# ssilverman16/particle_col_image_segmentation

Hardware: AMD Instinct MI355X
Metric: Mpixels/sec segmented (5-ch 1024x1024 TIFF), ROI mask IoU=1.0 (higher is better)
Workload: dtype f32 planes / u8 class maps / int32 labels / f64 ROI sums; 1 GPU; BASELINE config 2: batch of 64 frames 1024x1024x5 float32 per GPU, full kernel chain, inputs resident in HBM; frames_per_gpu=64, height=1024, width=1024, planes=5, parallelism=frames x1, launch=one hipGraph replay per step, 4 in flight, tie_fallback_frames_last_step=0, reference_nan_frames_rank0=0

## Files before the change

particle_col_image_segmentation_amd/csrc/ccl.hip:

```cpp
#include <type_traits>

#include "column_pass.h"
#include "tile_ops.h"

namespace pcseg {

constexpr int SCAN_PIX = 1024;

struct KeyEqU8 {
    const uint8_t *p;
    int W;
    int64_t n;
    __device__ __forceinline__ int operator()(int b, int r, int c) const { return p[b * n + rowoff(r, W) + c]; }
};
struct KeyNzU8 {
    const uint8_t *p;
    int W;
    int64_t n;
    __device__ __forceinline__ int operator()(int b, int r, int c) const { return p[b * n + rowoff(r, W) + c] != 0; }
};
struct KeyZeroU8 {
    const uint8_t *p;
    int W;
    int64_t n;
    __device__ __forceinline__ int operator()(int b, int r, int c) const { return p[b * n + rowoff(r, W) + c] == 0; }
};
struct KeyIsOneU8 {
    const uint8_t *p;
    int W;
    int64_t n;
    __device__ __forceinline__ int operator()(int b, int r, int c) const { return p[b * n + rowoff(r, W) + c] == 1; }
};
struct KeyI32 {
    const int32_t *p;
    int W;
    int64_t n;
    __device__ __forceinline__ int operator()(int b, int r, int c) const { return p[b * n + rowoff(r, W) + c]; }
};
__device__ __forceinline__ bool cand_bit(const unsigned long long *bits, int64_t g) { return (bits[g >> 6] >> (g & 63)) & 1ull; }
struct KeyCandBits {
    const int32_t *img;
    const unsigned long long *bits;
    int W;
    int64_t n;
    __device__ __forceinline__ int operator()(int b, int r, int c) const
    {
        const int64_t g = b * n + rowoff(r, W) + c;
        if (!cand_bit(bits, g)) return 0;
        const int v = img[g];
        return v == 0 ? (int)0x80000000 : v;
    }
};
struct KeyBits {
    const unsigned *words;
    int W, nch;
    __device__ __forceinline__ int operator()(int b, int r, int c) const
    {
        return (words[((int64_t)b * nch + (r >> 5)) * W + c] >> (r & 31)) & 1u;
    }
};

template <typename KeyFn, bool CONN8>
__global__ void __launch_bounds__(256) ccl_tile_kernel(KeyFn keyfn, int *__restrict__ parent, int H, int W)
{
    __shared__ int key[CCL_TILE];
    __shared__ int par[CCL_TILE];
    const int b = blockIdx.z, r0 = blockIdx.y * CCL_TH, c0 = blockIdx.x * CCL_TW;
    const int64_t fbase = (int64_t)b * H * W;
    if constexpr (std::is_same<KeyFn, KeyBits>::value) {
        const int lc = threadIdx.x % CCL_TW, c = c0 + lc;
        const unsigned word = c < W ? keyfn.words[((int64_t)b * keyfn.nch + (r0 >> 5)) * W + c] : 0u;
        for (int i = threadIdx.x; i < CCL_TILE; i += 256) {
            const int lr = i / CCL_TW;
            key[i] = (r0 + lr < H) ? (int)((word >> lr) & 1u) : 0;
        }
    } else {
        for (int i = threadIdx.x; i < CCL_TILE; i += 256) {
            int r = r0 + i / CCL_TW, c = c0 + i % CCL_TW;
            key[i] = (r < H && c < W) ? keyfn(b, r, c) : 0;
        }
    }
    __syncthreads();
    ccl_tile_unions<CONN8>(key, par);
    ccl_tile_store(key, par, parent, fbase, r0, c0, H, W);
}

template <typename KeyFn, bool CONN8>
__global__ void __launch_bounds__(256) ccl_border_kernel(KeyFn keyfn, int *__restrict__ parent, int H, int W, int *__restrict__ corrupt)
{
    const int n_top_rows = (H - 1) / CCL_TH, n_edges = (W - 1) / CCL_TW;
    const int n_cols = CONN8 ? 2 * n_edges : n_edges;
    int i = blockIdx.x * 256 + threadIdx.x;
    int r, c;
    if (i < n_top_rows * W) {
        r = (i / W + 1) * CCL_TH;
        c = i % W;
    } else {
        i -= n_top_rows * W;
        if (i >= n_cols * H) return;
        const int j = i / H;
        r = i % H;
        if ((r % CCL_TH) == 0 && r > 0) return;
        c = CONN8 ? ((j >> 1) + 1) * CCL_TW - (j & 1) : (j + 1) * CCL_TW;
    }
    const bool top = (r % CCL_TH) == 0 && r > 0;
    const bool left = (c % CCL_TW) == 0 && c > 0;
    const bool right = (c % CCL_TW) == CCL_TW - 1 && c + 1 < W;
    if (!top && !left && !(CONN8 && right && r > 0)) return;
    const int b = blockIdx.y;
    const int64_t fbase = (int64_t)b * H * W;
    int *par = parent + fbase;
    const int p = r * W + c;
    const int rn = max(r - 1, 0), cw = max(c - 1, 0), ce = min(c + 1, W - 1);
    const int k = keyfn(b, r, c);
    if (std::is_same<KeyFn, KeyCandBits>::value && k == 0) return;
    const int k_w = keyfn(b, r, cw), k_n = keyfn(b, rn, c), k_nw = keyfn(b, rn, cw), k_ne = CONN8 ? keyfn(b, rn, ce) : 0;
    if (k == 0) return;
    const bool w_same = c > 0 && k_w == k;
    const bool n_same = r > 0 && k_n == k;
    const bool nw_same = r > 0 && c > 0 && k_nw == k;
    const bool corner = top && left;
    int *bad = corrupt ? corrupt + b : nullptr;
    if (left && w_same && (corner || !(n_same && nw_same))) unite_glb(par, p, p - 1, bad);
    if (r > 0) {
        if (top && n_same && (corner || !(w_same && nw_same))) unite_glb(par, p, p - W, bad);
        if (CONN8) {
            if ((top || left) && nw_same && !n_same && !w_same) unite_glb(par, p, p - W - 1, bad);
            if (c + 1 < W && (top || right) && !n_same && k_ne == k) unite_glb(par, p, p - W + 1, bad);
        }
    }
}

struct PredAll {
    __device__ __forceinline__ bool operator()(int64_t) const { return true; }
};
struct PredNotFlagged {
    const uint8_t *flag;
    const int *frame_on;
    int64_t n;
    __device__ __forceinline__ bool operator()(int64_t gi) const { return flag[gi] == 0 && frame_on[gi / n] != 0; }
};

template <typename Pred>
__global__ void __launch_bounds__(256) ccl_flatten_count_kernel(int *__restrict__ parent, int *__restrict__ labels,
                                                                 int *__restrict__ blockcount, Pred pred, int64_t n, int nblk,
                                                                 bool flatten, int *__restrict__ corrupt)
{
    __shared__ int wsum[4];
    const int b = blockIdx.y;
    int *par = parent + (int64_t)b * n;
    int cnt = 0;
    const int64_t i0 = (int64_t)blockIdx.x * SCAN_PIX + threadIdx.x * 4;
    int pv[4] = {-1, -1, -1, -1};
    if ((n & 3) == 0 && i0 + 3 < n) {
        const int4 v = *reinterpret_cast<const int4 *>(par + i0);
        pv[0] = v.x; pv[1] = v.y; pv[2] = v.z; pv[3] = v.w;
    } else {
        for (int j = 0; j < 4; ++j)
            if (i0 + j < n) pv[j] = par[i0 + j];
    }
    bool isroot[4];
    for (int j = 0; j < 4; ++j) {
        const int64_t i = i0 + j;
        int p = pv[j];
        isroot[j] = false;
        if (i >= n || p < 0) continue;
        if (!walk_ok((int)i, p)) {
            walk_corrupt(corrupt ? corrupt + b : nullptr);
            continue;
        }
        if (flatten) {
            const int x = walk_root(par, p, corrupt ? corrupt + b : nullptr);
            if (x != p) par[i] = x;
            p = x;
        }
        isroot[j] = p == (int)i && pred((int64_t)b * n + i);
        cnt += isroot[j];
    }
    int total;
    int rank = block_exclusive_scan<256>(cnt, &total, wsum);
    for (int j = 0; j < 4; ++j)
        if (isroot[j]) labels[(int64_t)b * n + i0 + j] = -(++rank);
    if (threadIdx.x == 0) blockcount[b * nblk + blockIdx.x] = total;
}

__global__ void __launch_bounds__(256) ccl_scan_blocks_kernel(int *__restrict__ blockcount, int *__restrict__ counts, int nblk,
                                                               const int *__restrict__ corrupt)
{
    __shared__ int wsum[4];
    int *bc = blockcount + (int64_t)blockIdx.x * nblk;
    int carry = 0;
    for (int base = 0; base < nblk; base += 256) {
        int i = base + threadIdx.x;
        int v = i < nblk ? bc[i] : 0;
        int total;
        int ex = block_exclusive_scan<256>(v, &total, wsum);
        if (i < nblk) bc[i] = carry + ex;
        carry += total;
    }
    if (threadIdx.x == 0 && counts) counts[blockIdx.x] = (corrupt && corrupt[blockIdx.x]) ? -1 : carry;
}

template <typename Pred>
__global__ void __launch_bounds__(256) ccl_relabel_kernel(const int *__restrict__ parent, int *labels, const int *__restrict__ blockoff,
                                                           Pred pred, int64_t n, int nblk, bool chase, int *__restrict__ counts)
{
    const int b = blockIdx.y;
    const int *par = parent + (int64_t)b * n;
    int *lab = labels + (int64_t)b * n;
    const int64_t i0 = (int64_t)blockIdx.x * SCAN_PIX + threadIdx.x * 4;
    const bool vec = (n & 3) == 0 && i0 + 3 < n;
    int pv[4] = {-1, -1, -1, -1};
    if (vec) {
        const int4 v = *reinterpret_cast<const int4 *>(par + i0);
        pv[0] = v.x; pv[1] = v.y; pv[2] = v.z; pv[3] = v.w;
    } else {
        for (int j = 0; j < 4; ++j)
            if (i0 + j < n) pv[j] = par[i0 + j];
    }
    int out[4];
    int root_of_prev = -1, prev_p = -2;
    int bad = 0;
    for (int j = 0; j < 4; ++j) {
        int p = pv[j];
        int v = 0;
        if (p >= 0 && !walk_ok((int)(i0 + j), p)) {
            bad = 1;
            p = -1;
        }
        if (chase && p >= 0) {
            if (p == prev_p) {
                p = root_of_prev;
            } else {
                prev_p = p;
                p = walk_root(par, p, &bad);
                root_of_prev = p;
            }
        }
        if (p >= 0 && pred((int64_t)b * n + p)) {
            v = __hip_atomic_load(lab + p, __ATOMIC_RELAXED, __HIP_MEMORY_SCOPE_WORKGROUP);
            if (v < 0) v = blockoff[b * nblk + p / SCAN_PIX] - v;
        }
        out[j] = v;
    }
    if (vec) {
        *reinterpret_cast<int4 *>(lab + i0) = make_int4(out[0], out[1], out[2], out[3]);
    } else {
        for (int j = 0; j < 4; ++j)
            if (i0 + j < n) lab[i0 + j] = out[j];
    }
    if (bad && counts) counts[b] = -1;
}

constexpr int RELABEL_Q = 4;

template <typename Pred>
__device__ __forceinline__ int relabel_decode(const int *par, int *lab, const int *blockoff, const Pred &pred, int b, int64_t n, int nblk,
                                              int p, bool chase, int *bad)
{
    if (chase) p = walk_root(par, p, bad);
    if (!pred((int64_t)b * n + p)) return 0;
    int v = __hip_atomic_load(lab + p, __ATOMIC_RELAXED, __HIP_MEMORY_SCOPE_WORKGROUP);
    if (v < 0) v = blockoff[b * nblk + p / SCAN_PIX] - v;
    return v;
}

template <typename Pred, int NCH>
__device__ __forceinline__ void relabel_chains(const int *par, int *lab, const int *blockoff, const Pred &pred, int b, int64_t n, int nblk,
                                               bool chase, int (&root)[NCH], int (&val)[NCH], int *bad)
{
    if (chase) {
        bool more = true;
        while (more) {
            int nx[NCH];
#pragma unroll
            for (int q = 0; q < NCH; ++q) nx[q] = root[q] >= 0 ? par[root[q]] : -1;
            unsigned differ = 0, broke = 0;
#pragma unroll
            for (int q = 0; q < NCH; ++q) {
                const unsigned out = root[q] >= 0 && !walk_ok(root[q], nx[q]);
                broke |= out;
                nx[q] = out ? root[q] : nx[q];
                differ |= (unsigned)(nx[q] ^ root[q]);
// ... 23 lines not shown
{
    const int b = blockIdx.y;
    const int *par = parent + (int64_t)b * n;
    int *lab = labels + (int64_t)b * n;
    const int64_t i0 = (int64_t)blockIdx.x * (SCAN_PIX * RELABEL_Q) + threadIdx.x * 4;
    int4 pq[RELABEL_Q];
#pragma unroll
    for (int q = 0; q < RELABEL_Q; ++q) {
        const int64_t i = i0 + (int64_t)q * SCAN_PIX;
        pq[q] = i < n ? *reinterpret_cast<const int4 *>(par + i) : make_int4(-1, -1, -1, -1);
    }
    int bad = 0;
#pragma unroll
    for (int q = 0; q < RELABEL_Q; ++q) {
        const int i = (int)(i0 + (int64_t)q * SCAN_PIX);
        const int ox = pq[q].x >= 0 && !walk_ok(i, pq[q].x), oy = pq[q].y >= 0 && !walk_ok(i + 1, pq[q].y);
        const int oz = pq[q].z >= 0 && !walk_ok(i + 2, pq[q].z), ow = pq[q].w >= 0 && !walk_ok(i + 3, pq[q].w);
        bad |= ox | oy | oz | ow;
        pq[q].x = ox ? -1 : pq[q].x;
        pq[q].y = oy ? -1 : pq[q].y;
        pq[q].z = oz ? -1 : pq[q].z;
        pq[q].w = ow ? -1 : pq[q].w;
    }
    int lead[RELABEL_Q], lead2[RELABEL_Q], root[RELABEL_Q], val[RELABEL_Q], val2[RELABEL_Q], head_lane[RELABEL_Q];
    bool third = false;
    const int lane = lane_id();
#pragma unroll
    for (int q = 0; q < RELABEL_Q; ++q) {
        const int pv[4] = {pq[q].x, pq[q].y, pq[q].z, pq[q].w};
        lead[q] = pv[0] >= 0 ? pv[0] : (pv[1] >= 0 ? pv[1] : (pv[2] >= 0 ? pv[2] : pv[3]));
        const int left = __shfl_up(lead[q], 1);
        const bool head = lane == 0 || lead[q] != left;
        const unsigned long long heads = __ballot(head);
        head_lane[q] = 63 - __clzll((long long)(heads & (~0ull >> (63 - lane))));
        root[q] = head ? lead[q] : -1;
        lead2[q] = -1;
#pragma unroll
        for (int j = 1; j < 4; ++j) {
            if (pv[j] < 0 || pv[j] == lead[q]) continue;
            if (lead2[q] < 0) lead2[q] = pv[j];
            else if (pv[j] != lead2[q]) third = true;
        }
    }
    relabel_chains(par, lab, blockoff, pred, b, n, nblk, chase, root, val, &bad);
    bool any2 = false;
#pragma unroll
    for (int q = 0; q < RELABEL_Q; ++q) {
        val[q] = __shfl(val[q], head_lane[q]);
        root[q] = lead2[q];
        any2 = any2 || lead2[q] >= 0;
    }
    if (__any(any2)) relabel_chains(par, lab, blockoff, pred, b, n, nblk, chase, root, val2, &bad);
#pragma unroll
    for (int q = 0; q < RELABEL_Q; ++q) {
        const int64_t i = i0 + (int64_t)q * SCAN_PIX;
        if (i >= n) continue;
        const int pv[4] = {pq[q].x, pq[q].y, pq[q].z, pq[q].w};
        int out[4];
#pragma unroll
        for (int j = 0; j < 4; ++j) {
            out[j] = 0;
            if (pv[j] < 0) continue;
            if (pv[j] == lead[q]) out[j] = val[q];
            else if (pv[j] == lead2[q]) out[j] = val2[q];
            else if (third) out[j] = relabel_decode(par, lab, blockoff, pred, b, n, nblk, pv[j], chase, &bad);
        }
        *reinterpret_cast<int4 *>(lab + i) = make_int4(out[0], out[1], out[2], out[3]);
    }
    if (bad && counts) counts[b] = -1;
}

struct CclWs {
    int *parent;
    int *blockcount;
    int nblk;
    int *corrupt;
};

static CclWs ccl_carve(Carver &cv, int B, int H, int W)
{
    int64_t n = (int64_t)H * W;
    CclWs ws;
    ws.nblk = (int)((n + SCAN_PIX - 1) / SCAN_PIX);
    ws.parent = cv.take<int>((size_t)B * n);
    ws.blockcount = cv.take<int>((size_t)B * ws.nblk);
    ws.corrupt = cv.take<int>((size_t)B);
    return ws;
}

struct DilateCclWs {
    unsigned *bits, *dil;
};
static DilateCclWs dilate_ccl_carve(Carver &cv, int B, int H, int W)
{
    const size_t words = (size_t)B * ((H + 31) / 32) * W;
    DilateCclWs ws;
    ws.bits = cv.take<unsigned>(words);
    ws.dil = cv.take<unsigned>(words);
    return ws;
}
static unsigned *dilate_ccl_runs_carve(Carver &cv, int B, int H, int W) { return cv.take<unsigned>((size_t)B * ((H + 31) / 32) * W); }

struct FillHolesWs : CclWs {
    uint8_t *flag;
};
static FillHolesWs fill_holes_carve(Carver &cv, int B, int H, int W)
{
    FillHolesWs ws;
    static_cast<CclWs &>(ws) = ccl_carve(cv, B, H, W);
    ws.flag = cv.take<uint8_t>((size_t)B * H * W);
    return ws;
}

struct LocmaxWs : CclWs {
    size_t nwords;
    unsigned long long *cbits;
    uint8_t *bad;
    int *nonconst;
};
static LocmaxWs locmax_carve(Carver &cv, int B, int H, int W)
{
    const size_t total = (size_t)B * H * W;
    LocmaxWs ws;
    static_cast<CclWs &>(ws) = ccl_carve(cv, B, H, W);
    ws.nwords = (total + 63) / 64;
    ws.cbits = cv.take<unsigned long long>(ws.nwords + 1);
    ws.bad = cv.take<uint8_t>(total);
    ws.nonconst = cv.take<int>(B);
    return ws;
}

struct OverlapWs : CclWs {
    int *area, *ov;
};
static OverlapWs overlap_carve(Carver &cv, int B, int H, int W)
{
    OverlapWs ws;
    static_cast<CclWs &>(ws) = ccl_carve(cv, B, H, W);
    ws.area = cv.take<int>((size_t)B * H * W);
    ws.ov = cv.take<int>((size_t)B * H * W);
    return ws;
}

template <typename KeyFn, bool CONN8>
static int ccl_roots(KeyFn keyfn, int *parent, int B, int H, int W, hipStream_t s, bool tile_pass_done = false, int *corrupt = nullptr)
{
    if (corrupt) PCSEG_CHECK_HIP(hipMemsetAsync(corrupt, 0, sizeof(int) * (size_t)B, s));
    dim3 tgrid((W + CCL_TW - 1) / CCL_TW, (H + CCL_TH - 1) / CCL_TH, B);
    if (!tile_pass_done) {
        PCSEG_LAUNCH((ccl_tile_kernel<KeyFn, CONN8>), tgrid, dim3(256), 0, s, keyfn, parent, H, W);
        PCSEG_CHECK_LAUNCH();
    }
    if (tgrid.x > 1 || tgrid.y > 1) {
        const int64_t border_px = (int64_t)((H - 1) / CCL_TH) * W + (int64_t)(CONN8 ? 2 : 1) * ((W - 1) / CCL_TW) * H;
        dim3 bgrid((unsigned)((border_px + 255) / 256), B);
        PCSEG_LAUNCH((ccl_border_kernel<KeyFn, CONN8>), bgrid, dim3(256), 0, s, keyfn, parent, H, W, corrupt);
        PCSEG_CHECK_LAUNCH();
    }
    return PCSEG_OK;
}

template <typename Pred>
static int ccl_compact(int *parent, int *blockcount, int nblk, int *labels, int *counts, Pred pred, bool flatten,
                       int B, int H, int W, hipStream_t s, int *corrupt = nullptr)
{
    int64_t n = (int64_t)H * W;
    dim3 grid(nblk, B);
    PCSEG_LAUNCH((ccl_flatten_count_kernel<Pred>), grid, dim3(256), 0, s, parent, labels, blockcount, pred, n, nblk, false, corrupt);
    PCSEG_CHECK_LAUNCH();
    PCSEG_LAUNCH(ccl_scan_blocks_kernel, dim3(B), dim3(256), 0, s, blockcount, counts, nblk, (const int *)corrupt);
    PCSEG_CHECK_LAUNCH();
    if ((n & 3) == 0 && (((uintptr_t)parent | (uintptr_t)labels) & 15) == 0) {
        const dim3 qgrid((unsigned)((n + SCAN_PIX * RELABEL_Q - 1) / (SCAN_PIX * RELABEL_Q)), B);
        PCSEG_LAUNCH((ccl_relabel_quads_kernel<Pred>), qgrid, dim3(256), 0, s, (const int *)parent, labels, (const int *)blockcount, pred, n,
                     nblk, flatten, counts);
    } else {
        PCSEG_LAUNCH((ccl_relabel_kernel<Pred>), grid, dim3(256), 0, s, (const int *)parent, labels, (const int *)blockcount, pred, n, nblk,
                     flatten, counts);
    }
    PCSEG_CHECK_LAUNCH();
    return PCSEG_OK;
}

template <typename KeyFn, bool CONN8>
static int ccl_full(KeyFn keyfn, int32_t *labels, int32_t *counts, int B, int H, int W, void *workspace,
                    size_t workspace_bytes, hipStream_t s)
{
    Carver cv(workspace, workspace_bytes);
    CclWs ws = ccl_carve(cv, B, H, W);
    if (!cv.ok()) {
        set_error("ccl: workspace too small (%zu < %zu)", workspace_bytes, cv.off);
        return PCSEG_ERR_WORKSPACE;
    }
    int rc = ccl_roots<KeyFn, CONN8>(keyfn, ws.parent, B, H, W, s, false, ws.corrupt);
    if (rc) return rc;
    return ccl_compact(ws.parent, ws.blockcount, ws.nblk, labels, counts, PredAll(), true, B, H, W, s, ws.corrupt);
}

int ccl_plan(void *workspace, size_t workspace_bytes, int B, int H, int W, CclPlan *plan, const char *who)
{
    Carver cv(workspace, workspace_bytes);
    CclWs ws = ccl_carve(cv, B, H, W);
    if (!cv.ok()) {
        set_error("%s: workspace too small (%zu < %zu)", who, workspace_bytes, cv.off);
        return PCSEG_ERR_WORKSPACE;
    }
    plan->parent = ws.parent;
    plan->blockcount = ws.blockcount;
    plan->nblk = ws.nblk;
    plan->corrupt = ws.corrupt;
    return PCSEG_OK;
}

int ccl_equal_u8_finish(const uint8_t *in, const CclPlan &plan, bool tile_pass_done, int *labels, int *counts, int B, int H, int W,
                        hipStream_t s)
{
    const KeyEqU8 keyfn{in, W, (int64_t)H * W};
    PCSEG_CHECK_HIP(hipMemsetAsync(plan.corrupt, 0, sizeof(int) * (size_t)B, s));
    dim3 tgrid((W + CCL_TW - 1) / CCL_TW, (H + CCL_TH - 1) / CCL_TH, B);
    if (!tile_pass_done) {
        PCSEG_LAUNCH((ccl_tile_kernel<KeyEqU8, true>), tgrid, dim3(256), 0, s, keyfn, plan.parent, H, W);
        PCSEG_CHECK_LAUNCH();
    }
    if (tgrid.x > 1 || tgrid.y > 1) {
        const int64_t border_px = (int64_t)((H - 1) / CCL_TH) * W + (int64_t)2 * ((W - 1) / CCL_TW) * H;
        dim3 bgrid((unsigned)((border_px + 255) / 256), B);
        PCSEG_LAUNCH((ccl_border_kernel<KeyEqU8, true>), bgrid, dim3(256), 0, s, keyfn, plan.parent, H, W, plan.corrupt);
        PCSEG_CHECK_LAUNCH();
    }
    return ccl_compact(plan.parent, plan.blockcount, plan.nblk, labels, counts, PredAll(), true, B, H, W, s, plan.corrupt);
}

__global__ void __launch_bounds__(256) roots_to_parent_kernel(const int *__restrict__ roots, int *__restrict__ parent, int64_t total)
{
    int64_t i = (int64_t)blockIdx.x * blockDim.x + threadIdx.x;
    if (i < total) parent[i] = roots[i] - 1;
}

struct MaskSet {
    unsigned long long bits[4];
    int n;
};
template <bool VEC>
__global__ void __launch_bounds__(256) set_bits_kernel(const uint8_t *__restrict__ in, MaskSet masks, unsigned *__restrict__ bits,
                                                        int H, int W, int nch, int B)
{
    constexpr int COLS = VEC ? 4 : 1;
    const int c = (blockIdx.x * 256 + threadIdx.x) * COLS;
    const int ch = blockIdx.y, b = blockIdx.z;
    if (c >= W) return;
    const uint8_t *src = in + (int64_t)b * H * W + c;
    unsigned w[4][COLS];
#pragma unroll
    for (int m = 0; m < 4; ++m)
#pragma unroll
        for (int j = 0; j < COLS; ++j) w[m][j] = 0;
#pragma unroll 1
    for (int j0 = 0; j0 < 32; j0 += 8) {
        unsigned v8[8];
#pragma unroll
        for (int j = 0; j < 8; ++j) {
            const uint8_t *at = src + rowoff(min(ch * 32 + j0 + j, H - 1), W);
            v8[j] = VEC ? *reinterpret_cast<const unsigned *>(at) : (unsigned)*at;
        }
#pragma unroll
        for (int j = 0; j < 8; ++j) {
#pragma unroll
            for (int q = 0; q < COLS; ++q) {
                const unsigned a = (v8[j] >> (8 * q)) & 255u;
                const unsigned long long sel = a < 64 ? (1ull << a) : 0ull;
#pragma unroll
                for (int m = 0; m < 4; ++m)
                    if (m < masks.n && (masks.bits[m] & sel)) w[m][q] |= 1u << (j0 + j);
            }
        }
    }
    {
        const int rows = min(32, H - ch * 32);
        const unsigned valid = col_valid(rows);
#pragma unroll
        for (int m = 0; m < 4; ++m)
#pragma unroll
            for (int q = 0; q < COLS; ++q) w[m][q] &= valid;
    }
    const int64_t plane = (int64_t)B * nch * W;
#pragma unroll
    for (int m = 0; m < 4; ++m)
        if (m < masks.n) {
            unsigned *out = bits + m * plane + ((int64_t)b * nch + ch) * W + c;
            if constexpr (VEC) *reinterpret_cast<uint4 *>(out) = make_uint4(w[m][0], w[m][1], w[m][2], w[m][3]);
            else *out = w[m][0];
        }
}

__global__ void __launch_bounds__(256) dilate_bits_kernel(const unsigned *__restrict__ in, unsigned *__restrict__ out,
                                                           int radius, int H, int W, int nch)
{
    const int c = blockIdx.x * 256 + threadIdx.x;
    const int ch = blockIdx.y, b = blockIdx.z;
    if (c >= W) return;
    const unsigned *base = in + (int64_t)b * nch * W;
    unsigned acc = 0;
    for (int dy = 0; dy <= radius; ++dy) {
        int half = 0;
        while ((half + 1) * (half + 1) + dy * dy <= radius * radius) ++half;
        unsigned cur = 0, prev = 0, next = 0;
        for (int dx = -half; dx <= half; ++dx) {
            int cc = c + dx;
            if (cc < 0 || cc >= W) continue;
            cur |= base[rowoff(ch, W) + cc];
            if (dy > 0) {
                if (ch > 0) prev |= base[rowoff((ch - 1), W) + cc];
                if (ch + 1 < nch) next |= base[rowoff((ch + 1), W) + cc];
            }
        }
        if (dy == 0) acc |= cur;
        else {
            acc |= (cur << dy) | (prev >> (32 - dy));
            acc |= (cur >> dy) | (next << (32 - dy));
        }
    }
    const int rows = min(32, H - ch * 32);
    acc &= col_valid(rows);
    out[((int64_t)b * nch + ch) * W + c] = acc;
}

__global__ void __launch_bounds__(256) dilate_bits_disk2_kernel(const unsigned *__restrict__ in, unsigned *__restrict__ out, int H, int W,
                                                                 int nch)
{
    const int c = blockIdx.x * 256 + threadIdx.x;
    const int ch = blockIdx.y, b = blockIdx.z;
    if (c >= W) return;
    const unsigned *base = in + (int64_t)b * nch * W;
    const int chu = max(ch - 1, 0), chd = min(ch + 1, nch - 1);
    const unsigned *rc = base + rowoff(ch, W), *ru = base + rowoff(chu, W), *rd = base + rowoff(chd, W);
    const int c1l = max(c - 1, 0), c2l = max(c - 2, 0), c1r = min(c + 1, W - 1), c2r = min(c + 2, W - 1);
    const unsigned w0 = rc[c], w1l = rc[c1l], w1r = rc[c1r], w2l = rc[c2l], w2r = rc[c2r];
    unsigned u0 = ru[c], u1l = ru[c1l], u1r = ru[c1r], d0 = rd[c], d1l = rd[c1l], d1r = rd[c1r];
    if (ch == 0) u0 = u1l = u1r = 0;
    if (ch + 1 >= nch) d0 = d1l = d1r = 0;
    const unsigned cur1 = w0 | w1l | w1r, prev1 = u0 | u1l | u1r, next1 = d0 | d1l | d1r;
    unsigned acc = cur1 | w2l | w2r;
    acc |= (cur1 << 1) | (prev1 >> 31) | (cur1 >> 1) | (next1 << 31);
    acc |= (w0 << 2) | (u0 >> 30) | (w0 >> 2) | (d0 << 30);
    const int rows = min(32, H - ch * 32);
    acc &= col_valid(rows);
    out[((int64_t)b * nch + ch) * W + c] = acc;
}

constexpr int BR_TW = 64, BR_CH = 4, BR_ROWS = 32 * BR_CH;

__device__ __forceinline__ int bitrun_start(unsigned word, int p)
{
    const unsigned below = ~word & ((1u << p) - 1u);
    return below ? 32 - __clz(below) : 0;
}

template <typename Link>
__device__ __forceinline__ void bitrun_left_links(unsigned w, unsigned wl, Link &&link)
{
    unsigned rest = wl ? w : 0u;
    while (rest) {
        const int a = __ffs(rest) - 1;
        const unsigned from_a = w >> a;
        const int len = from_a == 0xFFFFFFFFu ? 32 : __ffs(~from_a) - 1;
        const int e = a + len - 1;
        rest = e >= 31 ? 0u : rest & ~((2u << e) - 1u);
        const int lo = max(a - 1, 0), hi = min(e + 1, 31);
        unsigned m = wl & (hi == 31 ? 0xFFFFFFFFu : ((2u << hi) - 1u)) & ~((1u << lo) - 1u);
        while (m) {
            const int p = __ffs(m) - 1;
            const int st = bitrun_start(wl, p);
            const unsigned from_p = wl >> p;
            const int run_len = from_p == 0xFFFFFFFFu ? 32 : __ffs(~from_p) - 1;
            const int en = p + run_len - 1;
            m = en >= 31 ? 0u : m & ~((2u << en) - 1u);
            link(a, st);
        }
    }
}

__global__ void __launch_bounds__(256) bitrun_tile_kernel(const unsigned *__restrict__ bits, int *__restrict__ parent, int H, int W,
                                                           int nch)
{
    __shared__ unsigned sw[BR_CH][BR_TW];
    __shared__ int lpar[BR_ROWS * BR_TW];
    const int col = threadIdx.x & (BR_TW - 1), q = threadIdx.x >> 6;
    const int c0 = blockIdx.x * BR_TW, ch0 = blockIdx.y * BR_CH, b = blockIdx.z;
    const int c = c0 + col, ch = ch0 + q;
    const unsigned w = (c < W && ch < nch) ? bits[((int64_t)b * nch + ch) * W + c] : 0u;
    sw[q][col] = w;
    for (unsigned heads = w & ~(w << 1); heads; heads &= heads - 1) {
        const int node = (q * 32 + (__ffs(heads) - 1)) * BR_TW + col;
        lpar[node] = node;
    }
    __syncthreads();
    if (w) {
        if (col > 0)
            bitrun_left_links(w, sw[q][col - 1], [&](int a, int st) {
                unite_lds(lpar, (q * 32 + a) * BR_TW + col, (q * 32 + st) * BR_TW + col - 1);
            });
        if ((w & 1u) && q > 0) {
            const int node = (q * 32) * BR_TW + col;
            const unsigned wu = sw[q - 1][col];
            if (wu >> 31) {
                unite_lds(lpar, node, ((q - 1) * 32 + bitrun_start(wu, 31)) * BR_TW + col);
            } else {
                if (col > 0 && (sw[q - 1][col - 1] >> 31))
                    unite_lds(lpar, node, ((q - 1) * 32 + bitrun_start(sw[q - 1][col - 1], 31)) * BR_TW + col - 1);
                if (col + 1 < BR_TW && (sw[q - 1][col + 1] >> 31))
                    unite_lds(lpar, node, ((q - 1) * 32 + bitrun_start(sw[q - 1][col + 1], 31)) * BR_TW + col + 1);
            }
        }
    }
    __syncthreads();
    int *par = parent + (int64_t)b * H * W;
    for (unsigned heads = w & ~(w << 1); heads; heads &= heads - 1) {
        const int node = (q * 32 + (__ffs(heads) - 1)) * BR_TW + col;
        const int root = find_lds(lpar, node);
        par[(ch0 * 32 + node / BR_TW) * W + c0 + node % BR_TW] = (ch0 * 32 + root / BR_TW) * W + c0 + root % BR_TW;
    }
}

__global__ void __launch_bounds__(256) bitrun_border_kernel(const unsigned *__restrict__ bits, int *__restrict__ parent, int H, int W,
                                                             int nch)
{
    const int c = blockIdx.x * 256 + threadIdx.x;
    const int ch = blockIdx.y, b = blockIdx.z;
    if (c >= W) return;
    const int col = c & (BR_TW - 1);
    const bool tile_left = col == 0 && c > 0, tile_top = (ch % BR_CH) == 0 && ch > 0;
    const bool edge_col = col == 0 || col == BR_TW - 1;
    if (!tile_left && !tile_top && !(edge_col && ch > 0)) return;
    const unsigned *wb = bits + (int64_t)b * nch * W;
    const int cl = c > 0 ? c - 1 : c, cr = c + 1 < W ? c + 1 : c, chu = ch > 0 ? ch - 1 : ch;
    const unsigned w = wb[rowoff(ch, W) + c], wl = wb[rowoff(ch, W) + cl];
    const unsigned wu = wb[rowoff(chu, W) + c], wul = wb[rowoff(chu, W) + cl], wur = wb[rowoff(chu, W) + cr];
    if (w == 0) return;
    int *par = parent + (int64_t)b * H * W;
    const int row0 = ch * 32;
    if (tile_left)
        bitrun_left_links(w, wl, [&](int a, int st) { unite_glb(par, (row0 + a) * W + c, (row0 + st) * W + c - 1); });
    if ((w & 1u) && ch > 0) {
        const int node = row0 * W + c;
        if (wu >> 31) {
            if (tile_top) unite_glb(par, node, (row0 - 32 + bitrun_start(wu, 31)) * W + c);
        } else {
            if (c > 0 && (tile_top || col == 0) && (wul >> 31)) unite_glb(par, node, (row0 - 32 + bitrun_start(wul, 31)) * W + c - 1);
            if (c + 1 < W && (tile_top || col == BR_TW - 1) && (wur >> 31))
                unite_glb(par, node, (row0 - 32 + bitrun_start(wur, 31)) * W + c + 1);
        }
    }
}

__global__ void __launch_bounds__(256) border_flag_kernel(const int *__restrict__ parent, uint8_t *__restrict__ flag, int H, int W)
{
    int t = blockIdx.x * blockDim.x + threadIdx.x;
    int r, c;
    if (t < W) { r = 0; c = t; }
    else if (t < 2 * W) { r = H - 1; c = t - W; }
    else if (t < 2 * W + H) { r = t - 2 * W; c = 0; }
    else if (t < 2 * W + 2 * H) { r = t - 2 * W - H; c = W - 1; }
    else return;
    int64_t fbase = (int64_t)blockIdx.y * H * W;
    int p = parent[fbase + rowoff(r, W) + c];
    if (p >= 0) flag[fbase + p] = 1;
}

__global__ void __launch_bounds__(256) fill_holes_out_kernel(const uint8_t *__restrict__ mask, const int *__restrict__ parent,
                                                              const uint8_t *__restrict__ flag, uint8_t *__restrict__ out, int64_t n)
{
    int64_t i = (int64_t)blockIdx.x * blockDim.x + threadIdx.x;
    if (i >= n) return;
    int64_t fbase = (int64_t)blockIdx.y * n;
    int p = parent[fbase + i];
    out[fbase + i] = (mask[fbase + i] != 0) || (p >= 0 && flag[fbase + p] == 0);
}

__global__ void __launch_bounds__(256) ccl_flatten_kernel(int *__restrict__ parent, int64_t n)
{
    int64_t i = (int64_t)blockIdx.x * blockDim.x + threadIdx.x;
    if (i >= n) return;
    int *par = parent + (int64_t)blockIdx.y * n;
    int p = par[i];
    if (p < 0 || !walk_ok((int)i, p)) return;
    const int x = walk_root(par, p);
    if (x != p) par[i] = x;
}

constexpr int LM_TW = CCL_TW, LM_TH = CCL_TH, LM_SW = LM_TW + 4, LM_SH = LM_TH + 4, LM_CW = LM_TW + 2, LM_CH = LM_TH + 2;

__global__ void __launch_bounds__(256) locmax_candidates_kernel(const int *__restrict__ img, unsigned long long *__restrict__ cbits,
                                                                 uint8_t *__restrict__ bad, int *__restrict__ nonconst,
                                                                 int *__restrict__ parent, int *__restrict__ markers, int H, int W)
{
    __shared__ int tile[LM_SH * LM_SW];
    __shared__ uint8_t cand[LM_CH * LM_CW];
    __shared__ int key[CCL_TILE];
    static_assert(LM_SH * LM_SW >= CCL_TILE, "the parents reuse the value tile");
    int *par = tile;
    const int OUTSIDE = (int)0x80000000;
    const TileIndex ti = xcd_tile_index();
    const int r0 = ti.y * LM_TH, c0 = ti.x * LM_TW;
    const int64_t fbase = (int64_t)ti.z * H * W;
    if ((W & 3) == 0 && c0 + LM_TW <= W && (((uintptr_t)img) & 15) == 0) {
        constexpr int QUADS = LM_SH * (LM_TW / 4), TRIPS = (QUADS + 255) / 256;
        int4 tq[TRIPS];
#pragma unroll
        for (int t = 0; t < TRIPS; ++t) {
            const int i = min((int)threadIdx.x + 256 * t, QUADS - 1);
            const int r = r0 + i / (LM_TW / 4) - 2;
            tq[t] = *reinterpret_cast<const int4 *>(img + fbase + rowoff(min(max(r, 0), H - 1), W) + c0 + 4 * (i % (LM_TW / 4)));
        }
        const int hl = min((int)threadIdx.x, LM_SH * 4 - 1);
        const int hr = r0 + (hl >> 2) - 2, hx = (hl & 3) < 2 ? (hl & 3) - 2 : LM_TW + (hl & 3) - 2, hc = c0 + hx;
        const int hv = img[fbase + rowoff(min(max(hr, 0), H - 1), W) + min(max(hc, 0), W - 1)];
#pragma unroll
        for (int t = 0; t < TRIPS; ++t) {
            const int i = (int)threadIdx.x + 256 * t;
            if (i < QUADS) {
                const int lr = i / (LM_TW / 4), r = r0 + lr - 2;
                const bool in = r >= 0 && r < H;
                int *dst = tile + lr * LM_SW + 2 + 4 * (i % (LM_TW / 4));
                dst[0] = in ? tq[t].x : OUTSIDE; dst[1] = in ? tq[t].y : OUTSIDE; dst[2] = in ? tq[t].z : OUTSIDE; dst[3] = in ? tq[t].w : OUTSIDE;
            }
        }
        if (threadIdx.x < LM_SH * 4) tile[(hl >> 2) * LM_SW + hx + 2] = (hr >= 0 && hr < H && hc >= 0 && hc < W) ? hv : OUTSIDE;
    } else {
        constexpr int TRIPS = (LM_SH * LM_SW + 255) / 256;
        int tv[TRIPS];
#pragma unroll
        for (int t = 0; t < TRIPS; ++t) {
            const int i = min((int)threadIdx.x + 256 * t, LM_SH * LM_SW - 1);
            const int r = r0 + i / LM_SW - 2, c = c0 + i % LM_SW - 2;
            tv[t] = img[fbase + rowoff(min(max(r, 0), H - 1), W) + min(max(c, 0), W - 1)];
        }
#pragma unroll
        for (int t = 0; t < TRIPS; ++t) {
            const int i = (int)threadIdx.x + 256 * t;
            const int r = r0 + i / LM_SW - 2, c = c0 + i % LM_SW - 2;
            if (i < LM_SH * LM_SW) tile[i] = (r >= 0 && r < H && c >= 0 && c < W) ? tv[t] : OUTSIDE;
        }
    }
    __syncthreads();
    const int first_value = img[fbase];
    bool any_differs = false;
    for (int t = threadIdx.x; t < LM_CH * LM_CW; t += 256) {
        const int lr = t / LM_CW, lc = t % LM_CW;
        const int r = r0 + lr - 1, c = c0 + lc - 1;
        const int i = (lr + 1) * LM_SW + lc + 1;
        const int v = tile[i];
        uint8_t state = 2;
        if (r >= 0 && r < H && c >= 0 && c < W) {
            const int *up = tile + i - LM_SW, *dn = tile + i + LM_SW;
            const int m = max(max(max(up[-1], up[0]), max(up[1], tile[i - 1])), max(max(tile[i + 1], dn[-1]), max(dn[0], dn[1])));
            state = m < v ? 1 : (m == v ? 3 : 0);
            any_differs = any_differs || v != first_value;
        }
        cand[t] = state;
    }
    __syncthreads();
    unsigned links = 0;
#pragma unroll
    for (int kk = 0; kk < LM_TH * LM_TW / 256; ++kk) {
        const int t = threadIdx.x + 256 * kk;
        const int lr = t / LM_TW, lc = t % LM_TW;
        const int r = r0 + lr, c = c0 + lc;
        int k = 0;
        if (r < H && c < W) {
            const int i = (lr + 2) * LM_SW + lc + 2, j = (lr + 1) * LM_CW + lc + 1;
            const int v = tile[i];
            const uint8_t st = cand[j];
            const bool is_cand = (st & 1) != 0;
            bool touches = false;
            if (st == 3) {
#pragma unroll
                for (int dr = -1; dr <= 1; ++dr)
#pragma unroll
                    for (int dc = -1; dc <= 1; ++dc) {
                        if (dr == 0 && dc == 0) continue;
                        const bool eq = tile[i + dr * LM_SW + dc] == v;
                        const uint8_t sn = cand[j + dr * LM_CW + dc];
                        touches = touches || (eq && sn == 0);
                        if ((dr < 0 || (dr == 0 && dc < 0)) && eq && (sn & 1) && lr + dr >= 0 && lc + dc >= 0 && lc + dc < LM_TW)
                            links |= 1u << (4 * kk + (dr == 0 ? 0 : dc + 2));
                    }
            }
            k = is_cand ? (v == 0 ? (int)0x80000000 : v) : 0;
            if (is_cand) bad[fbase + rowoff(r, W) + c] = touches ? 1 : 0;
            else if (markers) markers[fbase + rowoff(r, W) + c] = 0;
        }
        key[t] = k;
        const unsigned long long rowbits = __ballot(k != 0);
        if (lane_id() == 0 && r < H && rowbits) {
            const int64_t g = fbase + rowoff(r, W) + c0;
            const int sh = (int)(g & 63);
            atomicOr(cbits + (g >> 6), rowbits << sh);
            if (sh) atomicOr(cbits + (g >> 6) + 1, rowbits >> (64 - sh));
        }
    }
    if (__any(any_differs) && lane_id() == 0 && nonconst[ti.z] == 0) nonconst[ti.z] = 1;
    __syncthreads();
    for (int i = threadIdx.x; i < CCL_TILE; i += 256) par[i] = i;
    __syncthreads();
    if (links) {
// ... 411 lines not shown
```

particle_col_image_segmentation_amd/csrc/common.h:

```cpp
#pragma once
#include <hip/hip_runtime.h>
#include <stdint.h>
#include <stdio.h>
#include <string.h>

#include "../../include/pcseg.h"

namespace pcseg {

constexpr int WAVE = 64;

void set_error(const char *fmt, ...);

#define PCSEG_CHECK_HIP(expr)                                                              \
    do {                                                                                   \
        hipError_t _e = (expr);                                                            \
        if (_e != hipSuccess) {                                                            \
            pcseg::set_error("%s failed: %s (%s:%d)", #expr, hipGetErrorString(_e), __FILE__, __LINE__); \
            return PCSEG_ERR_HIP;                                                          \
        }                                                                                  \
    } while (0)

#define PCSEG_CHECK_LAUNCH()                                                               \
    do {                                                                                   \
// ... 107 lines not shown
}

struct TileIndex {
    int x, y, z;
};
__device__ __forceinline__ TileIndex xcd_tile_index()
{
    const unsigned gx = gridDim.x, gy = gridDim.y;
    const unsigned total = gx * gy * gridDim.z;
    const unsigned b = blockIdx.x + gx * (blockIdx.y + gy * blockIdx.z);
    const unsigned per = total / 8u;
    const unsigned t = b < per * 8u ? (b % 8u) * per + b / 8u : b;
    TileIndex ti;
    ti.x = (int)(t % gx);
    ti.y = (int)((t / gx) % gy);
    ti.z = (int)(t / (gx * gy));
    return ti;
}

__device__ __forceinline__ int ld_agent(const int *p)
{
    return __hip_atomic_load(p, __ATOMIC_RELAXED, __HIP_MEMORY_SCOPE_AGENT);
}
__device__ __forceinline__ unsigned ld_agent(const unsigned *p)
{
    return __hip_atomic_load(p, __ATOMIC_RELAXED, __HIP_MEMORY_SCOPE_AGENT);
}

__device__ __forceinline__ int ld_lds(const int *p) { return __hip_atomic_load(p, __ATOMIC_RELAXED, __HIP_MEMORY_SCOPE_WORKGROUP); }
__device__ __forceinline__ void st_lds(int *p, int v) { __hip_atomic_store(p, v, __ATOMIC_RELAXED, __HIP_MEMORY_SCOPE_WORKGROUP); }
__device__ __forceinline__ int find_lds(int *par, int x)
{
    int p;
    while ((p = ld_lds(par + x)) != x) x = p;
    return x;
}
__device__ __forceinline__ void unite_lds(int *par, int a, int b)
{
    for (;;) {
        a = find_lds(par, a);
        b = find_lds(par, b);
        if (a == b) return;
        if (a < b) { int t = a; a = b; b = t; }
        int old = atomicMin(&par[a], b);
        if (old == a) return;
        a = old;
    }
}
__device__ __forceinline__ void unite_lds_pair(int *par, int a, int b)
{
    for (;;) {
        for (;;) {
            if (a == b) return;
            const int pa = ld_lds(par + a), pb = ld_lds(par + b);
            if (pa == a && pb == b) break;
            a = pa;
            b = pb;
        }
        if (a < b) { int t = a; a = b; b = t; }
        int old = atomicMin(&par[a], b);
        if (old == a) return;
        a = old;
    }
}

__device__ __forceinline__ int find_lds_halving(int *par, int x)
{
    int p;
    while ((p = ld_lds(par + x)) != x) {
        const int g = ld_lds(par + p);
        if (g != p) st_lds(par + x, g);
        x = g;
    }
    return x;
}
__device__ __forceinline__ void unite_lds_halving(int *par, int a, int b)
{
    for (;;) {
        a = find_lds_halving(par, a);
        b = find_lds_halving(par, b);
        if (a == b) return;
        if (a < b) { int t = a; a = b; b = t; }
        const int old = atomicMin(&par[a], b);
        if (old == a) return;
        a = old;
    }
}

__device__ __forceinline__ bool walk_ok(int x, int p) { return (unsigned)p <= (unsigned)x; }
__device__ __forceinline__ void walk_corrupt(int *corrupt)
{
    if (corrupt) __hip_atomic_store(corrupt, 1, __ATOMIC_RELAXED, __HIP_MEMORY_SCOPE_AGENT);
}

__device__ __forceinline__ int walk_root(const int *par, int x, int *corrupt = nullptr)
{
    int q;
    while ((q = par[x]) != x) {
        if (!walk_ok(x, q)) {
            walk_corrupt(corrupt);
            break;
        }
        x = q;
    }
    return x;
}

__device__ __forceinline__ int find_glb(int *par, int x, int *corrupt = nullptr)
{
    int p;
    while ((p = ld_agent(par + x)) != x) {
        if (!walk_ok(x, p)) { walk_corrupt(corrupt); return x; }
        int g = ld_agent(par + p);
        if (!walk_ok(p, g)) { walk_corrupt(corrupt); return p; }
        if (g != p) __hip_atomic_store(par + x, g, __ATOMIC_RELAXED, __HIP_MEMORY_SCOPE_AGENT);
        x = g;
    }
    return x;
}
__device__ __forceinline__ bool find2_glb(int *par, int &a, int &b, int *corrupt = nullptr)
{
    for (;;) {
        if (a == b) return true;
        const int pa = ld_agent(par + a), pb = ld_agent(par + b);
        if (pa == a && pb == b) return true;
        if (!walk_ok(a, pa) || !walk_ok(b, pb)) break;
        const int ga = ld_agent(par + pa), gb = ld_agent(par + pb);
        if (!walk_ok(pa, ga) || !walk_ok(pb, gb)) break;
        if (pa != a) {
            if (ga != pa) __hip_atomic_store(par + a, ga, __ATOMIC_RELAXED, __HIP_MEMORY_SCOPE_AGENT);
            a = ga;
        }
        if (pb != b) {
            if (gb != pb) __hip_atomic_store(par + b, gb, __ATOMIC_RELAXED, __HIP_MEMORY_SCOPE_AGENT);
            b = gb;
        }
    }
    walk_corrupt(corrupt);
    return false;
}
__device__ __forceinline__ void unite_glb(int *par, int a, int b, int *corrupt = nullptr)
{
    for (;;) {
        if (!find2_glb(par, a, b, corrupt)) return;
        if (a == b) return;
        if (a < b) { int t = a; a = b; b = t; }
        int old = atomicMin(par + a, b);
        if (old == a) return;
        if (!walk_ok(a, old)) { walk_corrupt(corrupt); return; }
        a = old;
    }
}

struct CclPlan {
    int *parent;
    int *blockcount;
    int nblk;
    int *corrupt;
};
int ccl_plan(void *workspace, size_t workspace_bytes, int B, int H, int W, CclPlan *plan, const char *who);
int ccl_equal_u8_finish(const uint8_t *in, const CclPlan &plan, bool tile_pass_done, int *labels, int *counts, int B, int H, int W,
                        hipStream_t s);

}
```

Measured before the change: 17240 Mpixels/s.

## Compact border-link unions through shared-memory lists and per-seam border grid

The CCL border kernels are restructured. Each block first collects the union pairs it needs into a shared-memory list, using an atomic counter. After a barrier, the block's threads work through the compacted list, so the global union-find atomics are spread evenly instead of sitting in the few lanes that hit a tile edge. The border grid is also reshaped to one row of blocks per seam, replacing a flat index, which removes div/mod index math and keeps each block on one seam. The cost is extra LDS, two barriers and shared atomics per block, and the lists could overflow if capacity were wrong. Profiling helper scripts are added as well.

```diff
diff --git a/particle_col_image_segmentation_amd/csrc/ccl.hip b/particle_col_image_segmentation_amd/csrc/ccl.hip
--- a/particle_col_image_segmentation_amd/csrc/ccl.hip
+++ b/particle_col_image_segmentation_amd/csrc/ccl.hip
@@ -85,31 +85,13 @@
     ccl_tile_store(key, par, parent, fbase, r0, c0, H, W);
 }
 
-template <typename KeyFn, bool CONN8>
-__global__ void __launch_bounds__(256) ccl_border_kernel(KeyFn keyfn, int *__restrict__ parent, int H, int W, int *__restrict__ corrupt)
-{
-    const int n_top_rows = (H - 1) / CCL_TH, n_edges = (W - 1) / CCL_TW;
-    const int n_cols = CONN8 ? 2 * n_edges : n_edges;
-    int i = blockIdx.x * 256 + threadIdx.x;
-    int r, c;
-    if (i < n_top_rows * W) {
-        r = (i / W + 1) * CCL_TH;
-        c = i % W;
-    } else {
-        i -= n_top_rows * W;
-        if (i >= n_cols * H) return;
-        const int j = i / H;
-        r = i % H;
-        if ((r % CCL_TH) == 0 && r > 0) return;
-        c = CONN8 ? ((j >> 1) + 1) * CCL_TW - (j & 1) : (j + 1) * CCL_TW;
-    }
+template <typename KeyFn, bool CONN8, typename Link>
+__device__ __forceinline__ void ccl_border_links(const KeyFn &keyfn, int b, int r, int c, int H, int W, Link &&link)
+{
     const bool top = (r % CCL_TH) == 0 && r > 0;
     const bool left = (c % CCL_TW) == 0 && c > 0;
     const bool right = (c % CCL_TW) == CCL_TW - 1 && c + 1 < W;
     if (!top && !left && !(CONN8 && right && r > 0)) return;
-    const int b = blockIdx.y;
-    const int64_t fbase = (int64_t)b * H * W;
-    int *par = parent + fbase;
     const int p = r * W + c;
     const int rn = max(r - 1, 0), cw = max(c - 1, 0), ce = min(c + 1, W - 1);
     const int k = keyfn(b, r, c);
@@ -120,15 +102,51 @@
     const bool n_same = r > 0 && k_n == k;
     const bool nw_same = r > 0 && c > 0 && k_nw == k;
     const bool corner = top && left;
+    if (left && w_same && (corner || !(n_same && nw_same))) link(p, p - 1);
+    if (r > 0) {
+        if (top && n_same && (corner || !(w_same && nw_same))) link(p, p - W);
+        if (CONN8) {
+            if ((top || left) && nw_same && !n_same && !w_same) link(p, p - W - 1);
+            if (c + 1 < W && (top || right) && !n_same && k_ne == k) link(p, p - W + 1);
+        }
+    }
+}
+
+template <bool CONN8>
+static inline dim3 ccl_border_grid(int H, int W, int B)
+{
+    const int n_top = (H - 1) / CCL_TH, n_cols = (CONN8 ? 2 : 1) * ((W - 1) / CCL_TW);
+    const int row_len = n_top > 0 ? W : 0, col_len = n_cols > 0 ? H : 0, longest = row_len > col_len ? row_len : col_len;
+    return dim3((unsigned)((longest + 255) / 256), (unsigned)(n_top + n_cols), (unsigned)B);
+}
+template <typename KeyFn, bool CONN8>
+__global__ void __launch_bounds__(256) ccl_border_kernel(KeyFn keyfn, int *__restrict__ parent, int H, int W, int *__restrict__ corrupt)
+{
+    constexpr bool LIST = !std::is_same<KeyFn, KeyCandBits>::value;
+    __shared__ BlockLinks<2 * 256> links;
+    const int n_top_rows = (H - 1) / CCL_TH;
+    const int seam = blockIdx.y, at = blockIdx.x * 256 + threadIdx.x, b = blockIdx.z;
+    int r, c;
+    if (seam < n_top_rows) {
+        if (blockIdx.x * 256 >= W) return;
+        r = (seam + 1) * CCL_TH;
+        c = at;
+    } else {
+        if (blockIdx.x * 256 >= H) return;
+        const int j = seam - n_top_rows;
+        r = at;
+        c = CONN8 ? ((j >> 1) + 1) * CCL_TW - (j & 1) : (j + 1) * CCL_TW;
+        if ((r % CCL_TH) == 0 && r > 0) r = H;
+    }
+    int *par = parent + (int64_t)b * H * W;
     int *bad = corrupt ? corrupt + b : nullptr;
-    if (left && w_same && (corner || !(n_same && nw_same))) unite_glb(par, p, p - 1, bad);
-    if (r > 0) {
-        if (top && n_same && (corner || !(w_same && nw_same))) unite_glb(par, p, p - W, bad);
-        if (CONN8) {
-            if ((top || left) && nw_same && !n_same && !w_same) unite_glb(par, p, p - W - 1, bad);
-            if (c + 1 < W && (top || right) && !n_same && k_ne == k) unite_glb(par, p, p - W + 1, bad);
-        }
-    }
+    if (LIST) links_reset(links);
+    if (r < H && c < W)
+        ccl_border_links<KeyFn, CONN8>(keyfn, b, r, c, H, W, [&](int p, int q) {
+            if (LIST) links_push(links, p, q);
+            else unite_glb(par, p, q, bad);
+        });
+    if (LIST) links_unite(links, [&](int p, int q) { unite_glb(par, p, q, bad); });
 }
 
 struct PredAll {
@@ -458,9 +476,7 @@
         PCSEG_CHECK_LAUNCH();
     }
     if (tgrid.x > 1 || tgrid.y > 1) {
-        const int64_t border_px = (int64_t)((H - 1) / CCL_TH) * W + (int64_t)(CONN8 ? 2 : 1) * ((W - 1) / CCL_TW) * H;
-        dim3 bgrid((unsigned)((border_px + 255) / 256), B);
-        PCSEG_LAUNCH((ccl_border_kernel<KeyFn, CONN8>), bgrid, dim3(256), 0, s, keyfn, parent, H, W, corrupt);
+        PCSEG_LAUNCH((ccl_border_kernel<KeyFn, CONN8>), ccl_border_grid<CONN8>(H, W, B), dim3(256), 0, s, keyfn, parent, H, W, corrupt);
         PCSEG_CHECK_LAUNCH();
     }
     return PCSEG_OK;
@@ -529,9 +545,7 @@
         PCSEG_CHECK_LAUNCH();
     }
     if (tgrid.x > 1 || tgrid.y > 1) {
-        const int64_t border_px = (int64_t)((H - 1) / CCL_TH) * W + (int64_t)2 * ((W - 1) / CCL_TW) * H;
-        dim3 bgrid((unsigned)((border_px + 255) / 256), B);
-        PCSEG_LAUNCH((ccl_border_kernel<KeyEqU8, true>), bgrid, dim3(256), 0, s, keyfn, plan.parent, H, W, plan.corrupt);
+        PCSEG_LAUNCH((ccl_border_kernel<KeyEqU8, true>), ccl_border_grid<true>(H, W, B), dim3(256), 0, s, keyfn, plan.parent, H, W, plan.corrupt);
         PCSEG_CHECK_LAUNCH();
     }
     return ccl_compact(plan.parent, plan.blockcount, plan.nblk, labels, counts, PredAll(), true, B, H, W, s, plan.corrupt);
@@ -728,35 +742,40 @@
     }
 }
 
-__global__ void __launch_bounds__(256) bitrun_border_kernel(const unsigned *__restrict__ bits, int *__restrict__ parent, int H, int W,
-                                                             int nch)
-{
-    const int c = blockIdx.x * 256 + threadIdx.x;
-    const int ch = blockIdx.y, b = blockIdx.z;
-    if (c >= W) return;
+template <typename Link>
+__device__ __forceinline__ void bitrun_border_links(const unsigned *wb, int ch, int c, int W, Link &&link)
+{
     const int col = c & (BR_TW - 1);
     const bool tile_left = col == 0 && c > 0, tile_top = (ch % BR_CH) == 0 && ch > 0;
     const bool edge_col = col == 0 || col == BR_TW - 1;
     if (!tile_left && !tile_top && !(edge_col && ch > 0)) return;
-    const unsigned *wb = bits + (int64_t)b * nch * W;
     const int cl = c > 0 ? c - 1 : c, cr = c + 1 < W ? c + 1 : c, chu = ch > 0 ? ch - 1 : ch;
     const unsigned w = wb[rowoff(ch, W) + c], wl = wb[rowoff(ch, W) + cl];
     const unsigned wu = wb[rowoff(chu, W) + c], wul = wb[rowoff(chu, W) + cl], wur = wb[rowoff(chu, W) + cr];
     if (w == 0) return;
-    int *par = parent + (int64_t)b * H * W;
     const int row0 = ch * 32;
-    if (tile_left)
-        bitrun_left_links(w, wl, [&](int a, int st) { unite_glb(par, (row0 + a) * W + c, (row0 + st) * W + c - 1); });
+    if (tile_left) bitrun_left_links(w, wl, [&](int a, int st) { link((row0 + a) * W + c, (row0 + st) * W + c - 1); });
     if ((w & 1u) && ch > 0) {
         const int node = row0 * W + c;
         if (wu >> 31) {
-            if (tile_top) unite_glb(par, node, (row0 - 32 + bitrun_start(wu, 31)) * W + c);
+            if (tile_top) link(node, (row0 - 32 + bitrun_start(wu, 31)) * W + c);
         } else {
-            if (c > 0 && (tile_top || col == 0) && (wul >> 31)) unite_glb(par, node, (row0 - 32 + bitrun_start(wul, 31)) * W + c - 1);
-            if (c + 1 < W && (tile_top || col == BR_TW - 1) && (wur >> 31))
-                unite_glb(par, node, (row0 - 32 + bitrun_start(wur, 31)) * W + c + 1);
-        }
-    }
+            if (c > 0 && (tile_top || col == 0) && (wul >> 31)) link(node, (row0 - 32 + bitrun_start(wul, 31)) * W + c - 1);
+            if (c + 1 < W && (tile_top || col == BR_TW - 1) && (wur >> 31)) link(node, (row0 - 32 + bitrun_start(wur, 31)) * W + c + 1);
+        }
+    }
+}
+constexpr int BR_BLOCK_LINKS = 256 * 2 + (256 / BR_TW) * 31;
+__global__ void __launch_bounds__(256) bitrun_border_kernel(const unsigned *__restrict__ bits, int *__restrict__ parent, int H, int W,
+                                                             int nch)
+{
+    __shared__ BlockLinks<BR_BLOCK_LINKS> links;
+    const int c = blockIdx.x * 256 + threadIdx.x;
+    const int ch = blockIdx.y, b = blockIdx.z;
+    links_reset(links);
+    if (c < W) bitrun_border_links(bits + (int64_t)b * nch * W, ch, c, W, [&](int p, int q) { links_push(links, p, q); });
+    int *par = parent + (int64_t)b * H * W;
+    links_unite(links, [&](int p, int q) { unite_glb(par, p, q); });
 }
 
 __global__ void __launch_bounds__(256) border_flag_kernel(const int *__restrict__ parent, uint8_t *__restrict__ flag, int H, int W)
diff --git a/particle_col_image_segmentation_amd/csrc/common.h b/particle_col_image_segmentation_amd/csrc/common.h
--- a/particle_col_image_segmentation_amd/csrc/common.h
+++ b/particle_col_image_segmentation_amd/csrc/common.h
@@ -283,6 +283,32 @@
     }
 }
 
+template <int CAP>
+struct BlockLinks {
+    int n;
+    int2 pair[CAP];
+};
+template <int CAP>
+__device__ __forceinline__ void links_reset(BlockLinks<CAP> &l)
+{
+    if (threadIdx.x == 0) l.n = 0;
+    __syncthreads();
+}
+template <int CAP>
+__device__ __forceinline__ void links_push(BlockLinks<CAP> &l, int p, int q)
+{
+    l.pair[atomicAdd(&l.n, 1)] = make_int2(p, q);
+}
+template <int CAP, typename Unite>
+__device__ __forceinline__ void links_unite(BlockLinks<CAP> &l, Unite &&unite)
+{
+    __syncthreads();
+    const int n = l.n;
+    for (int i = threadIdx.x; i < n; i += blockDim.x) {
+        const int2 e = l.pair[i];
+        unite(e.x, e.y);
+    }
+}
 struct CclPlan {
     int *parent;
     int *blockcount;
diff --git a/profiles/border_links/resources.py b/profiles/border_links/resources.py
--- /dev/null
+++ b/profiles/border_links/resources.py
@@ -0,0 +1,30 @@
+import re
+import subprocess
+import sys
+
+FIELDS = [("VGPRs", r" VGPRs: (\d+)"), ("SGPRs", r"TotalSGPRs: (\d+)"), ("SGPR spill", r"SGPRs Spill: (\d+)"), ("LDS", r"LDS Size \[bytes/block\]: (\d+)"),
+          ("scratch", r"ScratchSize \[bytes/lane\]: (\d+)"), ("occupancy", r"Occupancy \[waves/SIMD\]: (\d+)")]
+
+
+def parse(paths):
+    out = {}
+    for path in paths.split(","):
+        for block in open(path).read().split("Function Name: ")[1:]:
+            name = block.split()[0]
+            if "border_kernel" in name:
+                out[name] = [re.search(rx, block).group(1) for _, rx in FIELDS]
+    return out
+
+
+def main():
+    a, b = parse(sys.argv[1]), parse(sys.argv[2])
+    names = sorted(set(a) | set(b))
+    plain = subprocess.run(["c++filt"] + names, capture_output=True, text=True).stdout.split("\n")
+    print("| Kernel | " + " | ".join(f for f, _ in FIELDS) + " |\n| --- |" + " --- |" * len(FIELDS))
+    for n, d in sorted(zip(names, plain), key=lambda t: t[1]):
+        d = re.sub(r"^void ", "", d).replace("pcseg::", "").split("(")[0]
+        cells = [x if x == y else "%s -> %s" % (x, y) for x, y in zip(a.get(n, ["-"] * len(FIELDS)), b.get(n, ["-"] * len(FIELDS)))]
+        print("| `%s` | %s |" % (d, " | ".join(cells)))
+
+
+main()
diff --git a/profiles/border_links/summarise.py b/profiles/border_links/summarise.py
--- /dev/null
+++ b/profiles/border_links/summarise.py
@@ -0,0 +1,83 @@
+import collections
+import csv
+import glob
+import json
+import os
+import statistics
+import sys
+
+KERNELS = ["ccl_border_kernel<pcseg::KeyEqU8, true>", "ws_uf_border_kernel", "bitrun_border_kernel", "ccl_border_kernel<pcseg::KeyCandBits, true>"]
+
+
+def kernel_of(name):
+    for k in KERNELS:
+        if k in name:
+            return k
+    return None
+
+
+def grid_of(r):
+    return int(r["Grid_Size_X"]) * int(r["Grid_Size_Y"]) * int(r["Grid_Size_Z"]) if "Grid_Size_X" in r else int(r["Grid_Size"])
+
+
+def trace_rows(out, side):
+    dur = collections.defaultdict(list)
+    for d in sorted(glob.glob(os.path.join(out, "trace_%s_*" % side))):
+        per = collections.defaultdict(list)
+        for p in glob.glob(os.path.join(d, "**", "*kernel_trace.csv"), recursive=True):
+            for r in csv.DictReader(open(p)):
+                k = kernel_of(r["Kernel_Name"])
+                if k:
+                    per[k].append((int(r["Start_Timestamp"]), (int(r["End_Timestamp"]) - int(r["Start_Timestamp"])) / 1e3, grid_of(r)))
+        for k, rows in per.items():
+            if k == "ws_uf_border_kernel":
+                top = max(g for _, _, g in rows)
+                groups = {k + " (first level)": [x for x in rows if x[2] == top], k + " (second level)": [x for x in rows if x[2] != top]}
+            else:
+                groups = {k: rows}
+            for name, g in groups.items():
+                g.sort()
+                dur[name] += [x[1] for x in g[len(g) // 4:]]
+    return dur
+
+
+def pmc_rows(out, side):
+    agg = collections.defaultdict(lambda: collections.defaultdict(float))
+    for p in glob.glob(os.path.join(out, "pmc_%s" % side, "**", "*counter_collection.csv"), recursive=True):
+        for r in csv.DictReader(open(p)):
+            k = kernel_of(r["Kernel_Name"])
+            if k:
+                agg[k][r["Counter_Name"]] += float(r["Counter_Value"])
+    return agg
+
+
+def main():
+    out = sys.argv[1]
+    a, b = trace_rows(out, "parent"), trace_rows(out, "branch")
+    if a or b:
+        print("| kernel | parent: launches, mean us (min .. max) | branch: launches, mean us (min .. max) | parent's spread | mean gain |\n| --- | --- | --- | --- | --- |")
+        for k in sorted(set(a) | set(b)):
+            cell = lambda v: "%d, %.1f (%.1f .. %.1f)" % (len(v), statistics.mean(v), min(v), max(v)) if v else "-"
+            gain = "%.1f" % (statistics.mean(a[k]) - statistics.mean(b[k])) if a[k] and b[k] else "-"
+            print("| `%s` | %s | %s | %s | %s |" % (k, cell(a[k]), cell(b[k]), "%.1f" % (max(a[k]) - min(a[k])) if a[k] else "-", gain))
+    runs = {s: [json.loads(open(p).read().strip().split("\n")[-1]) for p in sorted(glob.glob(os.path.join(out, "bench_%s_*.out" % s)))] for s in ("parent", "branch")}
+    if runs["parent"] or runs["branch"]:
+        print("\n| library | ms_per_step of the runs | median | range | config.launch |\n| --- | --- | --- | --- | --- |")
+        for s, rs in runs.items():
+            v = [r["ms_per_step"] for r in rs]
+            if v:
+                print("| %s | %s | %.3f | %.3f .. %.3f | %s |" % (s, " ".join("%.3f" % x for x in v), statistics.median(v), min(v), max(v),
+                                                               rs[0].get("config", {}).get("launch")))
+    pa, pb = pmc_rows(out, "parent"), pmc_rows(out, "branch")
+    if pa or pb:
+        print("\n| kernel | library | SQ_WAVE_CYCLES | SQ_WAIT_ANY | SQ_BUSY_CYCLES | SQ_WAIT_ANY / SQ_WAVE_CYCLES |\n| --- | --- | --- | --- | --- | --- |")
+        for k in KERNELS:
+            for s, t in (("parent", pa), ("branch", pb)):
+                c = t.get(k)
+                if c and c.get("SQ_WAVE_CYCLES"):
+                    print("| `%s` | %s | %.4g | %.4g | %.4g | %.2f |" % (k, s, c["SQ_WAVE_CYCLES"], c["SQ_WAIT_ANY"], c["SQ_BUSY_CYCLES"],
+                                                                   c["SQ_WAIT_ANY"] / c["SQ_WAVE_CYCLES"]))
+
+
+if __name__ == "__main__":
+    main()
```

Measured after the change: 16720 Mpixels/s. 0.97x the previous value.
